# genome/pindel

Measured on AMD Instinct MI355X. Metric: one-end-anchored reads/sec through split-read search (close end + far end), higher is better.
Workload: dtype u64; 1 GPU; BASELINE configs[2]: synthetic 10000000 x 100 bp one-end-anchored reads on a chr20-shaped reference (62435964 bp), all SV types (D/SI/TD/INV/none), Pindel defaults -x 2 -a 1 -m 3 -u 0.02 -e 0.01 -E 0.95 -H 8; reads_per_gpu=10000000, reads_total=10000000, read_len=100, insert_size=500, parallelism=reads sharded over 1 GPU(s) (weak scaling), reference replicated, no collective

## Files before the change

pindel_amd/csrc/pg_kernels.hip:

```cpp
#include <hip/hip_runtime.h>
#include <stdint.h>
#include <stdlib.h>

#include "pg_device.h"
#include "pg_lane_masks.h"
#include "pg_eval_masks.h"
#include "pg_fold_step.h"

typedef unsigned long long u64;
typedef unsigned int u32;
typedef u32 u32x4 __attribute__((ext_vector_type(4)));
typedef u32 u32x8 __attribute__((ext_vector_type(8)));

struct PgKArgs { PgDevRef ref; PgDevParams prm; PgDevBatch B; uint32_t max_len, levels; };
template <typename T> struct KaGlobal { static __device__ __forceinline__ T of(unsigned long long v) { return (T)v; } };
template <typename E> struct KaGlobal<E *> {
    static __device__ __forceinline__ E *of(unsigned long long v) { return (E *)(__attribute__((address_space(1))) E *)v; }
};
template <typename T>
__device__ __forceinline__ T karg_load(int off)
{
    const auto k = __builtin_amdgcn_kernarg_segment_ptr();
    if (sizeof(T) == 8) {
        unsigned long long v;
// ... 125 lines not shown
template <int NB, int NS, typename Id, int mode, bool DEF, bool EXACT, int LEN>
constexpr bool pg_short_fold()
{
    if (!pg_short_masks<NB, NS, mode, DEF, EXACT, LEN>() || sizeof(Id) != 4) return false;
    if (LEN > 0) return true;
    if (NB == 2 && NS == 3 && mode == PG_MODE_FAR) return false;
    if (NB == 4 && (mode == PG_MODE_BOTH || mode == PG_MODE_CLOSE)) return false;
    if (NB == 8 && NS == 4 && (mode == PG_MODE_CLOSE || mode == PG_MODE_FAR)) return false;
    return true;
}
template <int NB, int NS, typename Id, int mode, bool DEF, bool EXACT, int LEN>
constexpr bool pg_open_pass()
{
    return LEN > 0 && NB <= 2 && PG_PASS(NB) == 64 && DEF && !EXACT;
}
#define PG_QUEUE_IDLE(nb) ((uint16_t)((64u * (nb)) << 1))
__device__ __forceinline__ int count_below(u64 m)
{
    return (int)__builtin_amdgcn_mbcnt_hi((u32)(m >> 32), __builtin_amdgcn_mbcnt_lo((u32)m, 0u));
}
__device__ __forceinline__ u64 bit_range(int lo, int hi)
{
    return low_bits(hi) & ~low_bits(lo);
}
__device__ __forceinline__ u64 funnel64(u32 w0, u32 w1, u32 w2, u32 s)
{
    u32 a = __builtin_amdgcn_alignbit(w1, w0, s);
    u32 b = __builtin_amdgcn_alignbit(w2, w1, s);
    return (u64)a | ((u64)b << 32);
}
// ... 13 lines not shown
    asm("s_lshl_b32 %0, %4, %5\n\ts_lshr_b32 %1, %4, %6\n\ts_add_u32 %0, %0, %2\n\ts_addc_u32 %1, %1, %3"
        : "=&s"(lo), "=&s"(hi) : "s"(blo), "s"(bhi), "s"(r), "n"(SHIFT), "n"(32 - SHIFT) : "scc");
    return KaGlobal<T *>::of((u64)lo | ((u64)hi << 32));
}

template <typename Id> struct IdFmt;
template <> struct IdFmt<u32> { static constexpr int RB = PG_REL_BITS_SMALL; };
template <> struct IdFmt<u64> { static constexpr int RB = PG_REL_BITS; };
template <typename Id>
__device__ __forceinline__ Id make_id(u32 rel, bool isB, u32 region)
{
    return (Id)rel | ((Id)(isB ? 1u : 0u) << IdFmt<Id>::RB) | ((Id)region << (IdFmt<Id>::RB + 1));
}

enum { QP_LO = 0, QP_HI = 1, QP_NN = 2, QP_OO = 3 };

template <int NB>
struct Query {
    const u64 *qp;
    bool allowF_, allowB_;
    bool cF_, cB_;
    bool first_ok_;
    bool o1_;
    __device__ __forceinline__ bool allowF() const { return allowF_; }
    __device__ __forceinline__ bool allowB() const { return allowB_; }
    __device__ __forceinline__ bool cF() const { return cF_; }
    __device__ __forceinline__ bool cB() const { return cB_; }
    __device__ __forceinline__ bool first_ok() const { return first_ok_; }
};
template <int NB> __device__ __forceinline__ u64 q_lo(const Query<NB> &Q, int b) { return Q.qp[QP_LO * NB + b]; }
// ... 19 lines not shown
template <> struct AccB<u64> {
    typedef uint4 T;
    static __device__ __forceinline__ void load(const void *base, int i, u32 &m1, u32 &m2, u32 &ok, u64 &id)
    {
        const uint4 st = ((const uint4 *)base)[i];
        m1 = st.x; m2 = st.y & 0xffffu; ok = st.y >> 16; id = (u64)st.z | ((u64)st.w << 32);
    }
    template <bool SF>
    static __device__ __forceinline__ void store(void *base, int i, u32 m1, u32 m2, u32 ok, u64 id)
    {
        static_assert(!SF, "the short form of the fold step has 32-bit ids");
        ((uint4 *)base)[i] = make_uint4(m1, m2 | (ok << 16), (u32)id, (u32)(id >> 32));
    }
};

template <int NB, typename Id>
struct Lds {
    uint4 bufA[68];
    uint2 bufB[PG_PASS(NB) * NB];
    uint2 hdrB[64];
    u64 ringB[3 * NB];
    typename AccB<Id>::T accB[NB > 1 ? 64 * (NB - 1) : 1];
    u64 qp[2 * 4 * NB];
    uint16_t queue[PG_PASS(NB)];
    uint8_t mm_tab[PG_MM_IN_WIN(NB) ? 4 : 64 * NB + 64];
    uint2 chr_tab[PG_CHR_TAB_N(NB)];
#ifdef PG_TIMING
    u64 t_last;
    u32 t_acc[12];
    u32 t_pad[2];
#endif
    uint4 win[PG_WIN_STATIC_WORDS(NB)];
};

struct Search {
    int len, T, M, add_mm, bps, min_perfect, thr;
    uint16_t *queue;
    uint4 *win;
// ... 25 lines not shown
#define PG_STOP_AT(S, k) do { asm volatile("s_nop 14\n\ts_nop %0\n\ts_nop %1" : : "n"((k) & 7), "n"((k) >> 3)); \
                              if (PG_STOP == (k) && uni(opaque(1))) { (S).stopped = 1u; return; } } while (0)
#define PG_STOPPED(S) do { if ((S).stopped) return; } while (0)
#define PG_STOP_AT_V(S, k, v) do { asm volatile("s_nop 14\n\ts_nop %0\n\ts_nop %1" : : "n"((k) & 7), "n"((k) >> 3)); \
                                 if (PG_STOP == (k) && uni(opaque(1))) { (S).stopped = 1u; return (v); } } while (0)
#define PG_STOPPED_V(S, v) do { if ((S).stopped) return (v); } while (0)
#else
#define PG_STOP_AT(S, k) ((void)0)
#define PG_STOPPED(S) ((void)0)
#define PG_STOP_AT_V(S, k, v) ((void)0)
#define PG_STOPPED_V(S, v) ((void)0)
#endif
#ifdef PG_DIAG
    u32 dg;
#endif
#if defined(PG_DIAG) && PG_DIAG == 3
#define PG_DG(S, sh) ((void)0)
#define PG_DC(S, sh) ((void)0)
#define PG_DC_IF(S, cond, sh) ((void)0)
#define PG_DN(S, sh, n) (const_cast<Search &>(S).dg += (u32)(n) << (sh))
#elif defined(PG_DIAG) && PG_DIAG == 2
#define PG_DG(S, sh) ((void)0)
#define PG_DC(S, sh) ((S).dg += 1u << (sh))
#define PG_DC_IF(S, cond, sh) ((S).dg += (cond) ? 1u << (sh) : 0u)
#define PG_DN(S, sh, n) ((void)0)
#elif defined(PG_DIAG)
#define PG_DG(S, sh) ((S).dg += 1u << (sh))
#define PG_DC(S, sh) ((void)0)
#define PG_DC_IF(S, cond, sh) ((void)0)
#define PG_DN(S, sh, n) ((void)0)
#else
#define PG_DG(S, sh) ((void)0)
#define PG_DC(S, sh) ((void)0)
#define PG_DC_IF(S, cond, sh) ((void)0)
#define PG_DN(S, sh, n) ((void)0)
#endif
    int cap_state;
    u32 sf;
    __device__ __forceinline__ bool want_cap() const { return (sf & 1u) != 0u; }
    __device__ __forceinline__ bool tierA() const { return (sf & 2u) != 0u; }
    __device__ __forceinline__ bool len_check() const { return (sf & 4u) != 0u; }
};

template <int NB, typename Id>
struct Acc {
    u32 m1, m2, ok;
    Id id;
    u32 a1, a2, aok;
    Id aid;
    u32 dirty;
    template <bool SF>
// ... 38 lines not shown
template <int NB>
__device__ __forceinline__ int chr_size_of(const PgDevRef &ref, const Search &S, int c)
{
    if (c < PG_CHR_TAB_N(NB)) {
        const int sz = uni((int)S.chr_tab[c].y);
        if (sz != 0) return sz;
    }
    return uni((int)KA(ref, chr_size)[c]);
}

template <int NB>
__device__ __forceinline__ void block_masks(const Query<NB> &Q, int b, bool comp,
                                            u64 rlo, u64 rhi, u64 rnn, u64 &mis, u64 &qn)
{
    const u64 qlo = q_lo<NB>(Q, b), qhi = q_hi<NB>(Q, b), qnn = q_nn<NB>(Q, b), qoo = q_oo<NB>(Q, b);
    u64 cm = comp ? ~0ull : 0ull;
    u64 x = rlo ^ qlo ^ cm;
    u64 y = rhi ^ qhi ^ cm;
    u64 d = x | y;
    mis = (d & ~qnn) | rnn | qoo;
    qn = qnn;
}

__device__ __forceinline__ void fetch_lds(const uint4 *win, int wbase, int q, bool rev,
                                          u64 &rlo, u64 &rhi, u64 &rnn)
{
    u32 rel = (u32)(q - wbase);
    u32 wi = rel >> 5, s = rel & 31u;
    uint4 w0 = win[wi], w1 = win[wi + 1], w2 = win[wi + 2];
    rlo = funnel64(w0.x, w1.x, w2.x, s);
    rhi = funnel64(w0.y, w1.y, w2.y, s);
    rnn = funnel64(w0.z, w1.z, w2.z, s);
    if (rev) { rlo = __brevll(rlo); rhi = __brevll(rhi); rnn = __brevll(rnn); }
}
__device__ __forceinline__ void fetch_lds_uniform(const uint4 *win, int wbase, int q, bool rev,
                                                  u64 &rlo, u64 &rhi, u64 &rnn)
// ... 75 lines not shown
            }
            u32 okc = pg_fs_verdict_b<SF>(bad, h.y);
            if (!SF && S.len_check()) okc = (u32)L >= ((h.y >> 24) & 0x7fu) ? okc : 0u;
            const Id cid = sizeof(Id) == 8 ? (Id)((u64)h.x | ((u64)(h.y & 0xffffffu) << 32)) : (Id)h.x;
            fold<Id>(m1, m2, wid, ok, k, cid, okc);
        }
        if (r == 0) { A.m1 = m1; A.m2 = m2; A.ok = ok; A.id = wid; }
        else {
            AccB<Id>::template store<SF>(S.accB, (r - 1) * 64 + lB, m1, m2, ok, wid);
            PG_DN(S, 27, 1);
            A.dirty |= 1u << r;
        }
    }
}

template <int NB, typename Id, bool MIXED, bool SM, bool SF, bool OP>
__device__ __forceinline__ void fold_candidates(const Search &S, const Query<NB> &Q, Acc<NB, Id> &A, int wbase,
                                                int origin, u32 region, int n, int lane, const Rings &R, int *ring_n)
{
    constexpr int EW = NB;
    PG_DG(const_cast<Search &>(S), 16);
    const u64 inm = low_bits(n);
    int p = 0;
    bool isB = MIXED ? false : Q.allowB();
    if (OP) {
        static_assert(!OP || PG_PASS(NB) == WAVE, "the open pass: one queue slot and one bufB slot per lane");
        const u32 e = S.queue[lane];
        if (MIXED) isB = e & 1u;
        p = wbase + (int)(e >> 1);
    } else if (lane_bit(inm)) {
        u32 e = S.queue[lane];
        if (MIXED) isB = e & 1u;
        p = wbase + (int)(e >> 1);
    }
    const bool comp = isB ? Q.cB() : Q.cF();
    int cum = 0, lvl0 = 0, kA = 0;
    int kk[NB];
    u32 m0lo = 0u, s0lo = 0u;
#pragma unroll
    for (int r = 0; r < NB; r++) kk[r] = 0;
    u64 needm = inm;
    const int alive = S.T > S.thr ? S.T : S.thr;
#pragma unroll
    for (int b = 0; b < NB; b++) {
        if (64 * b >= S.len) break;
        if (needm == 0ull) break;
        if (OP || lane_bit(needm)) {
            u64 rlo, rhi, rnn, m, s;
            int q = isB ? p - 64 * b - 63 : p + 64 * b;
            if (MIXED) fetch_lds(S.win, wbase, q, isB, rlo, rhi, rnn);
            else fetch_lds_uniform(S.win, wbase, q, isB, rlo, rhi, rnn);
            block_masks<NB>(Q, b, comp, rlo, rhi, rnn, m, s);
            const u64 lm = low_bits(S.len - 64 * b);
            m &= lm;
            s = (m ^ s) & lm;
            S.bufB[lane * EW + b] = make_uint2((u32)m, (u32)(m >> 32));
            cum += __popcll(m);
            if (b == 0) {
                lvl0 = __popcll(m & low_bits(S.bps));
                kA = __popc((u32)m & low32(S.bps + 16));
                m0lo = (u32)m;
                s0lo = (u32)s;
            }
#pragma unroll
            for (int r = 1; r < NB; r++)
                if (b <= r) kk[r] += __popcll(m & low_bits(S.bps + 64 * r - 64 * b));
        }
// ... 561 lines not shown
    PG_DG(const_cast<Search &>(S), 8);
    if (NS <= 4 && (S.ro & PG_RO_OK)) {
        constexpr int RNS = NS <= 3 ? 3 : 4;
        if (DUAL) seed_filter_ro<NB, 2, RNS>(S, Q.o1_, wide, lane, mF, mB);
        else if (kindB) seed_filter_ro<NB, 1, RNS>(S, Q.o1_, wide, lane, mF, mB);
        else seed_filter_ro<NB, 0, RNS>(S, Q.o1_, wide, lane, mF, mB);
        return;
    }
    const u32 jmask = S.jmask[wide ? 1 : 0];
    const u32 g0mask = jmask & low32(S.bps);
    int cap0 = (int)((S.depth >> (wide ? 24 : 16)) & 0xffu);
    if (cap0 > S.cap_state) cap0 = S.cap_state;
    seed_filter_run<NB, NS, DUAL>(S, Q, kindB, lane, jmask, g0mask, cap0, mF, mB);
}

template <int NB, int NS, typename Id, bool MIXED, bool W3, bool SM, bool SF, bool OP>
__device__ __forceinline__ void scan_impl(const PgDevRef &ref, Search &S,
                                          const Query<NB> &Q, Acc<NB, Id> &A, long long wo, int g0, int s, int e,
                                          int e_max, int xs, int xe, int origin, u32 region, int lane,
                                          u32 use_cache, u32 &cacheF, u32 &cacheB, u32 &cache_valid)
{
    if (!Q.first_ok() || s >= e) return;
    PG_STOP_AT(S, 33);
    const int k0 = (s - g0) >> PG_CHUNK_SHIFT, k1 = (e - 1 - g0) >> PG_CHUNK_SHIFT;
    for (int k = k0; k <= k1; k++) {
        const int cs = g0 + (k << PG_CHUNK_SHIFT);
        const int ns = s > cs ? s : cs;
        {
            const int ne = e < cs + (int)PG_CHUNK ? e : cs + (int)PG_CHUNK;
            if (ns >= xs && ne <= xe) continue;
        }
// ... 38 lines not shown
                    h++;
                    if (ballot64((mF | mB) != 0u) == 0ull) continue;
                    const u32 cnt = (u32)(__popc(mF) + __popc(mB));
                    const u32 incl = wave_scan(cnt);
                    slot = end + (int)(incl - cnt);
                    end += (int)read_lane(incl, 63);
                    pos0 = (u32)(64 * NB + 32 * word);
                    continue;
                }
                else if (end > 0) n = end;
                else break;
                S.nsurv += n;
                S.nsurv_total += (u32)n;
                PG_SYNC();
                PG_T(S, S.t_base);
                fold_candidates<NB, Id, MIXED, SM, SF, OP>(S, Q, A, wb, origin, region, n, lane, Rings{ false, 0, 0, 0, 0 }, nullptr);
                PG_STOPPED(S);
                PG_T(S, S.t_base + 1);
                slot -= n;
                end -= n;
                if (end == 0 && h == nh) break;
            }
            k += nh - 1;
            continue;
        }
        const int ne = e < cs + (int)PG_CHUNK ? e : cs + (int)PG_CHUNK;
        const int se = e_max < cs + (int)PG_CHUNK ? e_max : cs + (int)PG_CHUNK;
        PG_STOP_AT(S, 34);
        if (!(wo == S.win_wo && S.wbase == wb && se + 64 * NB <= S.win_hi))
            stage_window<NB>(ref, S, wo, wb, se + 64 * NB, lane);
        PG_STOP_AT(S, 13);
// ... 33 lines not shown
                S.queue[slot - base] = (uint16_t)((u32)(64 * NB + 32 * lane + bit) << 1);
                slot++;
            }
            while (mF == 0u && mB != 0u && slot < top) {
                const int bit = __ffs((int)mB) - 1;
                mB &= mB - 1u;
                S.queue[slot - base] = (uint16_t)(((u32)(64 * NB + 32 * lane + bit) << 1) | 1u);
                slot++;
            }
            const int n = total - base < PG_PASS(NB) ? total - base : PG_PASS(NB);
            S.nsurv += n;
            S.nsurv_total += (u32)n;
            PG_SYNC();
            PG_T(S, S.t_base);
            PG_STOP_AT(S, 16);
            fold_candidates<NB, Id, MIXED, SM, SF, OP>(S, Q, A, wb, origin, region, n, lane, Rings{ false, 0, 0, 0, 0 }, nullptr);
            PG_STOPPED(S);
            PG_T(S, S.t_base + 1);
        }
    }
}

template <int NB, int NS, typename Id, bool W3, bool SM, bool SF, bool OP>
__device__ __forceinline__ void scan_range(const PgDevRef &ref, Search &S,
                                           const Query<NB> &Q, Acc<NB, Id> &A, long long wo, int g0, int s, int e,
                                           int e_max, int xs, int xe, int origin, u32 region, int lane,
                                           u32 use_cache, u32 &cacheF, u32 &cacheB, u32 &cache_valid)
{
    g0 = uni(g0); s = uni(s); e = uni(e); e_max = uni(e_max); xs = uni(xs); xe = uni(xe); origin = uni(origin);
    if (Q.allowF() && Q.allowB())
        scan_impl<NB, NS, Id, true, W3, SM, SF, OP>(ref, S, Q, A, wo, g0, s, e, e_max, xs, xe, origin, region, lane,
                                    use_cache, cacheF, cacheB, cache_valid);
    else
        scan_impl<NB, NS, Id, false, false, SM, SF, OP>(ref, S, Q, A, wo, g0, s, e, e_max, xs, xe, origin, region, lane,
                                        use_cache, cacheF, cacheB, cache_valid);
}

template <int NB, int NS, typename Id, bool SM, bool SF, bool OP>
__device__ __forceinline__ void scan_staged(Search &S, const Query<NB> &Q, Acc<NB, Id> &A, int g0, int s, int e, int origin,
                                            int lane, u32 keep, u32 &cacheF, u32 &cacheB, u32 &cache_valid)
{
    const int wb = g0 - 64 * NB;
    PG_STOP_AT(S, 33);
    PG_STOP_AT(S, 34);
    PG_STOP_AT(S, 13);
    PG_STOP_AT(S, 37);
    u32 mF = 0u, mB = 0u, unused;
    if (Q.allowB()) seed_filter<NB, NS, false>(S, Q, true, false, lane, mB, unused);
    else seed_filter<NB, NS, false>(S, Q, false, false, lane, mF, unused);
    if (keep) { cacheF = mF; cacheB = mB; cache_valid = 1u; }
    PG_STOP_AT(S, 14);
    const u32 kb = Q.allowB() ? 1u : 0u;
    const int pbase = g0 + 32 * lane;
// ... 6 lines not shown
    for (int base = 0; base < total; base += PG_PASS(NB)) {
        PG_SYNC();
        const int top = base + PG_PASS(NB);
        while (m != 0u && slot < top) {
            const int bit = __ffs((int)m) - 1;
            m &= m - 1u;
            S.queue[slot - base] = (uint16_t)(((u32)(64 * NB + 32 * lane + bit) << 1) | kb);
            slot++;
        }
        const int n = total - base < PG_PASS(NB) ? total - base : PG_PASS(NB);
        S.nsurv += n;
        S.nsurv_total += (u32)n;
        PG_SYNC();
        PG_T(S, S.t_base);
        PG_STOP_AT(S, 16);
        fold_candidates<NB, Id, false, SM, SF, OP>(S, Q, A, wb, origin, 0u, n, lane, Rings{ false, 0, 0, 0, 0 }, nullptr);
        PG_STOPPED(S);
        PG_T(S, S.t_base + 1);
    }
}

struct RegionInfo {
    int chr;
    int origin;
    const pg_window *bd;
};

template <int NB, typename Id>
struct Eval {
    Id id[NB];
    u32 lo[NB];
    u64 startm[NB], brkm[NB];
    int n_runs, max_len;
    Id id_last;
};

template <int NB>
__device__ __forceinline__ u32 mm_of(const Search &S, int L)
{
    if (PG_MM_IN_WIN(NB)) return (S.win[L >> 2].w >> (8 * (L & 3))) & 0xffu;
    return S.mm_tab[L];
}

template <int NB, typename Id, bool SE, bool SF>
__device__ __forceinline__ void evaluate(Search &S, const Acc<NB, Id> &A, Eval<NB, Id> &E, int lane, int qmask = 15)
{
    static_assert(PG_MM_BREAKS < 64, "the short form's reach rule: no level of a point reaches 64");
    const u32 mm0 = mm_of<NB>(S, S.bps + lane);
    E.n_runs = 0;
    E.max_len = 0;
    E.id_last = 0;
    PG_DG(S, 24);
    u32 t1 = A.m1, t2 = A.m2, tok = A.ok;
    Id tid = A.id;
    if (S.tierA()) {
        u32 a1 = PG_BIG, a2 = PG_BIG, aok = pg_fs_none<SF>();
        Id aid = 0;
        if (lane < 16) { a1 = A.a1; a2 = A.a2; aok = A.aok; aid = A.aid; }
        if (qmask != 1) {
            PG_DC(S, 24);
            if (SF) S.bufA[lane] = make_uint4(A.a1, A.a2, (u32)A.aid, A.aok);
            else S.bufA[lane] = make_uint4(A.a1, A.a2 | (A.aok << 16), (u32)A.aid, (u32)((u64)A.aid >> 32));
            PG_SYNC();
            if (lane < 16) {
#pragma unroll
                for (int q = 1; q < 4; q++) {
                    if (!((qmask >> q) & 1)) continue;
                    const uint4 o = S.bufA[lane + 16 * q];
                    const Id oid = sizeof(Id) == 8 ? (Id)((u64)o.z | ((u64)o.w << 32)) : (Id)o.z;
                    if (SF) merge<Id>(a1, a2, aid, aok, o.x, o.y, oid, o.w);
// ... 115 lines not shown
            dst[0] = isB ? (u32)(p - L + 1) : (u32)(p + L - 1);
            dst[1] = (u32)L | ((u32)(S.bps + 64 * r + end_lane) << 16);
            dst[2] = E.lo[r] | ((isB ? PG_RUN_BACKWARD : 0u) << 8) | ((anti ? PG_RUN_ANTISENSE : 0u) << 8) |
                     ((u32)(chr & 0xffff) << 16);
        }
        written += __popcll(kept[r]);
    }
}

template <int NB>
__device__ __forceinline__ u64 request_planes(const PgDevBatch &B, uint32_t rid, int lane)
{
    const u32 pb = KA(B, plane_blocks);
    return (u32)lane < 8u * pb ? KA(B, planes)[(size_t)rid * 8u * pb + (u32)lane] : 0ull;
}
template <int NB>
__device__ __forceinline__ void store_planes(const PgDevBatch &B, u64 v, int lane, u64 *qp)
{
    const u32 pb = KA(B, plane_blocks);
    PG_SYNC();
    if ((u32)lane < 8u * pb) qp[pb == (u32)NB ? (u32)lane : ((u32)lane / pb) * NB + (u32)lane % pb] = v;
    PG_SYNC();
}

__device__ __forceinline__ u32 pool_alloc(const PgDevBatch &B, int n, int lane, u32 &fits)
{
    const u32 shard = blockIdx.x & (PG_POOL_SHARDS - 1u);
    u32 off = 0;
    if (n > 0 && lane == 0) off = atomicAdd(KA(B, pool_used) + shard * 16u, (u32)n);
    off = (u32)uni((int)off);
    fits = (u64)off + (u64)n <= (u64)KA(B, pool_shard_cap) ? 1u : 0u;
    return shard * KA(B, pool_shard_cap) + off;
}

template <int NB, int NS, typename Id, int mode, bool DEF, bool EXACT = false, int LEN = 0>
__device__ __forceinline__ void search_read(const PgDevRef &ref, const PgDevParams &prm, const PgDevBatch &B,
                                            Search &S, u64 *qplanes, const uint32_t rid, const int touch_next, const int lane,
                                            const u32 res_base, const u32 res_fits)
{
    constexpr bool OP = pg_open_pass<NB, NS, Id, mode, DEF, EXACT, LEN>();
#define PG_LANE (NB <= 2 && !OP ? lane_now() : opaque(lane))
    S.win_wo = -1;
    S.win_hi = S.wbase = 0;
    S.nsurv_total = 0u;
#ifdef PG_TIMING
    S.t_base = 1;
#endif
#ifdef PG_DIAG
    S.dg = 0u;
#endif
    S.cap_state = 255;
    S.sf = 0u;
#ifdef PG_STOP
    S.stopped = 0u;
#endif
// ... 32 lines not shown
        S.thr = (int)(F.lvl & 0xffffu);
        S.M = (int)((F.lvl >> 16) & 0xffu);
        S.T = (int)(F.lvl >> 24);
        S.depth = F.depth;
        S.jmask[0] = F.jmask0;
        S.ro = F.ro;
    }
    S.rid = rid;
    S.rp_lo = (u32)uni((int)(u32)(u64)(uintptr_t)rp);
    S.rp_hi = (u32)uni((int)(u32)((u64)(uintptr_t)rp >> 32));
    PG_STOP_AT(S, 10);
    if ((mode & PG_MODE_CLOSE) && (flags & PG_RF_CLOSE_OK)) {
        const int ss = (int)ra[2], se = (int)ra[3];
        if (ss < se) stage_window<NB>(ref, S, chr_wo, ss - 64 * NB, se + 64 * NB, lane, rp + uni(touch_next));
    }
    store_planes<NB>(B, planes_of_read, lane, qplanes);

    PG_T(S, 0);
#if defined(PG_STOP) && PG_STOP == 1
    if (uni(opaque(1))) return;
#endif
    int ja = 0, jb = 0, ex_stage = 0;
    auto ex_apply = [&](int to) __attribute__((always_inline)) {
        while (ex_stage < to) {
            ex_stage++;
            const int cut = ex_stage == 1 ? ja : jb;
            u64 *pl = qplanes + (ex_stage == 1 ? 0 : 4 * NB);
            if (cut > 0) {
                const int l = PG_LANE;
                u64 v = 0ull;
                if (l < 4 * NB) {
// ... 90 lines not shown
                    A.template reset<SF>();
                    S.cap_state = 255;
                    S.nsurv = 0;
                    nsurv_eval = 0;
                    ps = pe = 0;
                }
                if (att == 1 || att == 3) {
                    const u32 t0 = cr0, t1 = cr1;
                    const u32 tv = vr;
                    cr0 = co0; cr1 = co1; vr = vo;
                    co0 = t0; co1 = t1; vo = tv;
                }
                const bool own_grid = att == 0 && !shared_grid;
                PG_STOP_AT_V(S, 12, true);
                if (staged)
                    scan_staged<NB, NS, Id, SM, SF, OP>(S, Q, A, own_grid ? s1 : w1s, s1, e1, w1s, PG_LANE, shared_grid, cr0, cr1, vr);
                else
                scan_range<NB, NS, Id, !DEF, SM, SF, OP>(ref, S, Q, A, chr_wo, own_grid ? s1 : w1s, s1, e1, own_grid ? e1 : w1e, ps, pe, w1s, 0u,
                                   PG_LANE, (att == 1 || att == 2 ? 1u : 0u) | shared_grid, cr0, cr1, vr);
                PG_STOPPED_V(S, true);
                PG_STOP_AT_V(S, 19, true);
                ps = s1;
                pe = e1;
                if (S.nsurv != nsurv_eval) {
                    nsurv_eval = S.nsurv;
                    Eval<NB, Id> E;
                    PG_DC(S, 0);
                    evaluate<NB, Id, SE, SF>(S, A, E, PG_LANE);
                    PG_STOP_AT_V(S, 20, true);
                    close_max = uni(E.max_len);
                    if (uni(E.n_runs) > 0) {
                        u64 kept[NB];
                        n_close = uni(count_kept<NB, Id, SE>(E, true, kept));
                        if (n_close <= (int)PG_RES_CLOSE) {
                            close_base = res_base;
                            fits = res_fits;
                        } else
                            close_base = pool_alloc(B, n_close, lane, fits);
                        PG_DC(S, 20);
                        if (fits) emit_runs<NB, Id, SE>(S, true, false, chr, w1s, nullptr, E, kept, KA(B, pool) + close_base, PG_LANE);
                        const u64 idl = (u64)E.id_last;
                        const int pl = w1s + (int)(u32)(idl & ((1ull << IdFmt<Id>::RB) - 1ull));
                        close_last = ((idl >> IdFmt<Id>::RB) & 1ull) ? (u32)(pl - close_max + 1) : (u32)(pl + close_max - 1);
// ... 49 lines not shown
        Q.qp = qplanes + (flipped ? 4 * NB : 0);
        Q.o1_ = flipped != 0;
        Q.cF_ = flipped; Q.cB_ = !flipped;
        Q.allowF_ = Q.allowB_ = true;
        Q.first_ok_ = (flags & (flipped ? PG_RF_FIRST_OK_REV : PG_RF_FIRST_OK_FWD)) != 0u;
        if (Q.first_ok_) {
            u32x4 rc;
            asm volatile("s_load_dwordx4 %0, %1, 0x30\n\ts_waitcnt lgkmcnt(0)" : "=&s"(rc) : "s"(record_ptr<7>(KA(B, in), rid)));
            const int chr_size = (int)rc[0];
            S.jmask[1] = LEN > 0 ? pg_fixed_len_row((uint32_t)LEN).jmask1 : rc[3];
            PG_STOP_AT(S, 35);
            int far_bases = 0;
            auto far_update = [&](int origin, const pg_window *bdw, int qmask) {
                Eval<NB, Id> E;
                PG_DC(S, 4);
                evaluate<NB, Id, SE, SF>(S, A, E, PG_LANE, qmask);
                const int mx = uni(E.max_len);
                if (mx >= far_max) {
                    far_max = mx;
                    n_far = uni(E.n_runs);
                    far_base = 0;
                    if (n_far > 0) {
                        u64 kept[NB];
                        (void)count_kept<NB, Id, SE>(E, false, kept);
                        if (n_far <= (int)PG_RES_FAR) {
                            far_base = res_base + PG_RES_CLOSE;
                            fits &= res_fits;
                        } else {
                            u32 f2 = 1u;
                            far_base = pool_alloc(B, n_far, lane, f2);
                            fits &= f2;
// ... 6 lines not shown
            bool done = false;
            const pg_window *bd_all = KA(B, bd);
            if (bd_all && rc[1] != 0u) {
                const int nbd = (int)rc[1];
                const pg_window *bd = bd_all + rc[2];
                A.template reset<SF>();
                S.cap_state = 255;
                S.nsurv = 0;
                for (int w = 0; w < nbd; w++) {
                    const pg_window bw = bd[w];
                    const int st = bw.start < 0 ? bw.end - 1 : bw.start;
                    const bool own_chr = uni(bw.chr_id) == chr;
                    const int csz = own_chr ? chr_size : chr_size_of<NB>(ref, S, uni(bw.chr_id));
                    const int s = st < 0 ? 0 : st, e = bw.end > csz ? csz : bw.end;
                    far_bases += (e > s ? e - s : 0) + 2 * len;
                    scan_range<NB, NS, Id, !DEF, SM, SF, OP>(ref, S, Q, A, own_chr ? chr_wo : chr_word_off_of<NB>(ref, S, uni(bw.chr_id)), s, s, e, e, 0, 0, st,
                                       (u32)w, PG_LANE, false, unused0, unused1, unused_valid);
                    PG_STOPPED(S);
                }
                if (S.nsurv > 0) far_update(0, bd, 15);
                done = far_max + close_max >= len;
            }
            if (!done) {
                const int center = (int)close_last;
                const int k_mri = PRM(max_range_index, PG_DEF_MAX_RANGE_INDEX);
                const u32 k_spacer = PRM(spacer, PG_DEF_SPACER);
                const int maxspan = 64 << (2 * k_mri);
                const int origin = center - maxspan;
                const int g0 = center - (int)PG_CHUNK / 2;
                const u32 reach = (u32)maxspan + k_spacer;
                const bool noclip = reach >= k_spacer && (u32)center > reach && (u32)chr_size > reach && (u32)center < (u32)chr_size - reach;
// ... 59 lines not shown
                                    S.queue[slot] = (uint16_t)((u32)(64 * NB + 32 * lane + bit) << 1);
                                    slot++;
                                }
                                while (mB != 0u) {
                                    const int bit = __ffs((int)mB) - 1;
                                    mB &= mB - 1u;
                                    S.queue[slot] = (uint16_t)(((u32)(64 * NB + 32 * lane + bit) << 1) | 1u);
                                    slot++;
                                }
                                S.nsurv += total;
                                S.nsurv_total += (u32)total;
                                PG_SYNC();
                                PG_STOP_AT(S, 27);
                                int ring_n[3];
                                PG_T(S, 7);
                                fold_candidates<NB, Id, true, SM, SF, OP>(S, Q, A, wb, origin, 0u, total, lane,
                                                              Rings{ true, rs[0], re[0], rs[1], re[1] }, ring_n);
                                PG_STOPPED(S);
                                PG_STOP_AT(S, 30);
                                PG_T(S, 8);
                                for (int r = 0; r <= R; r++) {
                                    if (uni(ring_n[r]) > 0) {
                                        u64 longm[NB];
#pragma unroll
                                        for (int k = 0; k < NB; k++) longm[k] = read_lane(S.ringB[r * NB + k], 0);
                                        fold_tier_b<NB, Id, SM, SF>(S, Q, A, longm, lane);
                                        far_update(origin, nullptr, r == 0 ? 1 : (r == 1 ? 3 : 15));
                                    }
                                    if (far_max + close_max >= len) {
                                        done = true;
                                        ps = rs[r];
                                        pe = re[r];
                                        break;
                                    }
                                }
                                nsurv_eval = S.nsurv;
                            }
                        }
                    }
                    PG_STOP_AT(S, 31);
                }
                int span = 64 << (2 * r_first);
                for (int r = r_first; r <= k_mri && !done; r++, span *= 4) {
                    int s, e;
                    range_of(span, s, e);
                    if (s < e) {
                        scan_range<NB, NS, Id, !DEF, SM, SF, OP>(ref, S, Q, A, chr_wo, g0, s, e, emax, ps, pe, origin, 0u, PG_LANE, true,
                                           cacheF, cacheB, cache_valid);
                        PG_STOPPED(S);
                        if (ps < pe) {
                            ps = s < ps ? s : ps;
                            pe = e > pe ? e : pe;
                        } else {
                            ps = s; pe = e;
                        }
                    }
                    if (S.nsurv != nsurv_eval) {
                        nsurv_eval = S.nsurv;
                        far_update(origin, nullptr, 15);
                    }
                    if (far_max + close_max >= len) break;
                }
// ... 736 lines not shown
```

pindel_amd/csrc/pg_search_kernel_body.h:

```cpp
    __shared__ Lds<NB, Id> lds;
    const int lane = threadIdx.x;
    if (PG_WIN_DYN_BYTES(NB) != 0u) {
        extern __shared__ uint4 pg_dyn_lds[];
        if ((const char *)pg_dyn_lds != (const char *)&lds + sizeof(lds)) __builtin_trap();
    }
    if (PG_MM_IN_WIN(NB)) {
        for (int w = lane; w < 16 * NB + 16; w += WAVE) {
            u32 v = 0u;
#pragma unroll
            for (int k = 0; k < 4; k++) v |= (u32)max_mismatch_at(prm.mm_bp, 4 * w + k) << (8 * k);
            lds.win[w].w = v;
        }
    } else
        for (int L = lane; L < 64 * NB + 64; L += WAVE) lds.mm_tab[L] = (uint8_t)max_mismatch_at(prm.mm_bp, L);
    if (lane < PG_CHR_TAB_N(NB) && lane < ref.n_chr) {
        const u64 wo = ref.chr_word_off[lane];
        lds.chr_tab[lane] = make_uint2((u32)wo, (wo >> 32) == 0ull ? ref.chr_size[lane] : 0u);
    }
    PG_SYNC();
    Search S;
    S.queue = lds.queue;
    S.win = lds.win;
    S.bufA = lds.bufA;
    S.bufB = lds.bufB;
    S.hdrB = lds.hdrB;
    S.ringB = lds.ringB;
    S.accB = lds.accB;
    S.mm_tab = lds.mm_tab;
    S.chr_tab = lds.chr_tab;
    u64 *qplanes = lds.qp;
    if (lane < 8 * NB) qplanes[lane] = 0ull;
    if (pg_open_pass<NB, NS, Id, mode, DEF, false, LEN>() && lane < PG_PASS(NB)) lds.queue[lane] = PG_QUEUE_IDLE(NB);
#ifdef PG_TIMING
    S.t_acc = lds.t_acc;
    S.t_last = &lds.t_last;
    if (lane == 0) {
        for (int k = 0; k < 12; k++) S.t_acc[k] = 0u;
        *S.t_last = __builtin_readcyclecounter();
    }
    S.t_base = 1;
#endif

    uint32_t part = blockIdx.x % PG_N_XCD, tried = 0;
    while (tried < PG_N_XCD) {
        const uint32_t n = KA(B, n_reads);
        const uint32_t claim = KA(B, claim);
// ... 44 lines not shown
```

Before: 581.9 million reads/s.

## Precompute bit-reversed query planes and tree-merge quarter accumulators in evaluate

After: 588.2 million reads/s (median of 6 runs). 1.01x the previous value.

```diff
diff --git a/pindel_amd/csrc/pg_kernels.hip b/pindel_amd/csrc/pg_kernels.hip
--- a/pindel_amd/csrc/pg_kernels.hip
+++ b/pindel_amd/csrc/pg_kernels.hip
@@ -6,6 +6,7 @@
 #include "pg_lane_masks.h"
 #include "pg_eval_masks.h"
 #include "pg_fold_step.h"
+#include "pg_pass_forms.h"
 
 typedef unsigned long long u64;
 typedef unsigned int u32;
@@ -163,6 +164,16 @@
 {
     return LEN > 0 && NB <= 2 && PG_PASS(NB) == 64 && DEF && !EXACT;
 }
+template <int NB, int NS, typename Id, int mode, bool DEF, bool EXACT, int LEN>
+constexpr bool pg_rev_mismatch()
+{
+    return LEN > 0 && NB == 2 && DEF && !EXACT;
+}
+template <int NB, int NS, typename Id, int mode, bool DEF, bool EXACT, int LEN>
+constexpr bool pg_tree_merge()
+{
+    return LEN > 0 && NB <= 2 && PG_PASS(NB) == 64 && pg_short_fold<NB, NS, Id, mode, DEF, EXACT, LEN>();
+}
 #define PG_QUEUE_IDLE(nb) ((uint16_t)((64u * (nb)) << 1))
 __device__ __forceinline__ int count_below(u64 m)
 {
@@ -206,6 +217,7 @@
 }
 
 enum { QP_LO = 0, QP_HI = 1, QP_NN = 2, QP_OO = 3 };
+#define PG_QP_REV(nb) (2 * 4 * (nb))
 
 template <int NB>
 struct Query {
@@ -255,14 +267,14 @@
     }
 };
 
-template <int NB, typename Id>
+template <int NB, typename Id, int QPX = 2>
 struct Lds {
     uint4 bufA[68];
     uint2 bufB[PG_PASS(NB) * NB];
     uint2 hdrB[64];
     u64 ringB[3 * NB];
     typename AccB<Id>::T accB[NB > 1 ? 64 * (NB - 1) : 1];
-    u64 qp[2 * 4 * NB];
+    u64 qp[QPX * 4 * NB];
     uint16_t queue[PG_PASS(NB)];
     uint8_t mm_tab[PG_MM_IN_WIN(NB) ? 4 : 64 * NB + 64];
     uint2 chr_tab[PG_CHR_TAB_N(NB)];
@@ -318,7 +330,13 @@
 #ifdef PG_DIAG
     u32 dg;
 #endif
-#if defined(PG_DIAG) && PG_DIAG == 3
+#if defined(PG_DIAG) && PG_DIAG == 4
+#define PG_DG(S, sh) ((void)0)
+#define PG_DC(S, sh) ((void)0)
+#define PG_DC_IF(S, cond, sh) ((void)0)
+#define PG_DN(S, sh, n) ((void)0)
+#define PG_DK(S, sh) (const_cast<Search &>(S).dg += 1u << (sh))
+#elif defined(PG_DIAG) && PG_DIAG == 3
 #define PG_DG(S, sh) ((void)0)
 #define PG_DC(S, sh) ((void)0)
 #define PG_DC_IF(S, cond, sh) ((void)0)
@@ -339,6 +357,9 @@
 #define PG_DC_IF(S, cond, sh) ((void)0)
 #define PG_DN(S, sh, n) ((void)0)
 #endif
+#ifndef PG_DK
+#define PG_DK(S, sh) ((void)0)
+#endif
     int cap_state;
     u32 sf;
     __device__ __forceinline__ bool want_cap() const { return (sf & 1u) != 0u; }
@@ -407,12 +428,24 @@
                                             u64 rlo, u64 rhi, u64 rnn, u64 &mis, u64 &qn)
 {
     const u64 qlo = q_lo<NB>(Q, b), qhi = q_hi<NB>(Q, b), qnn = q_nn<NB>(Q, b), qoo = q_oo<NB>(Q, b);
-    u64 cm = comp ? ~0ull : 0ull;
-    u64 x = rlo ^ qlo ^ cm;
-    u64 y = rhi ^ qhi ^ cm;
-    u64 d = x | y;
-    mis = (d & ~qnn) | rnn | qoo;
+    mis = pg_pf_mismatch(rlo, rhi, rnn, qlo, qhi, qnn, qoo, comp);
     qn = qnn;
+}
+template <int NB>
+__device__ __forceinline__ void block_masks_at(const Query<NB> &Q, const u64 *qb, int b, bool comp,
+                                               u64 rlo, u64 rhi, u64 rnn, u64 &mis, u64 &qn)
+{
+    mis = pg_pf_mismatch(rlo, rhi, rnn, qb[QP_LO * NB + b], qb[QP_HI * NB + b], qb[QP_NN * NB + b], qb[QP_OO * NB + b], comp);
+    qn = q_nn<NB>(Q, b);
+}
+__device__ __forceinline__ void fetch_lds_plain(const uint4 *win, int wbase, int q, u64 &rlo, u64 &rhi, u64 &rnn)
+{
+    u32 rel = (u32)(q - wbase);
+    u32 wi = rel >> 5, s = rel & 31u;
+    uint4 w0 = win[wi], w1 = win[wi + 1], w2 = win[wi + 2];
+    rlo = funnel64(w0.x, w1.x, w2.x, s);
+    rhi = funnel64(w0.y, w1.y, w2.y, s);
+    rnn = funnel64(w0.z, w1.z, w2.z, s);
 }
 
 __device__ __forceinline__ void fetch_lds(const uint4 *win, int wbase, int q, bool rev,
@@ -518,7 +551,7 @@
     }
 }
 
-template <int NB, typename Id, bool MIXED, bool SM, bool SF, bool OP>
+template <int NB, typename Id, bool MIXED, bool SM, bool SF, bool OP, bool RM>
 __device__ __forceinline__ void fold_candidates(const Search &S, const Query<NB> &Q, Acc<NB, Id> &A, int wbase,
                                                 int origin, u32 region, int n, int lane, const Rings &R, int *ring_n)
 {
@@ -538,6 +571,7 @@
         p = wbase + (int)(e >> 1);
     }
     const bool comp = isB ? Q.cB() : Q.cF();
+    const u64 *const qrm = Q.qp + (RM && isB ? PG_QP_REV(NB) : 0);
     int cum = 0, lvl0 = 0, kA = 0;
     int kk[NB];
     u32 m0lo = 0u, s0lo = 0u;
@@ -549,12 +583,23 @@
     for (int b = 0; b < NB; b++) {
         if (64 * b >= S.len) break;
         if (needm == 0ull) break;
+        PG_DK(S, MIXED ? 12 : (isB ? 0 : 6));
         if (OP || lane_bit(needm)) {
             u64 rlo, rhi, rnn, m, s;
             int q = isB ? p - 64 * b - 63 : p + 64 * b;
+            if (RM) {
+                fetch_lds_plain(S.win, wbase, q, rlo, rhi, rnn);
+                block_masks_at<NB>(Q, qrm, b, comp, rlo, rhi, rnn, m, s);
+                if (MIXED) m = isB ? __brevll(m) : m;
+                else if (uni((int)isB)) {
+                    asm volatile("" : "+v"(m));
+                    m = __brevll(m);
+                }
+            } else {
             if (MIXED) fetch_lds(S.win, wbase, q, isB, rlo, rhi, rnn);
             else fetch_lds_uniform(S.win, wbase, q, isB, rlo, rhi, rnn);
             block_masks<NB>(Q, b, comp, rlo, rhi, rnn, m, s);
+            }
             const u64 lm = low_bits(S.len - 64 * b);
             m &= lm;
             s = (m ^ s) & lm;
@@ -1146,7 +1191,7 @@
     seed_filter_run<NB, NS, DUAL>(S, Q, kindB, lane, jmask, g0mask, cap0, mF, mB);
 }
 
-template <int NB, int NS, typename Id, bool MIXED, bool W3, bool SM, bool SF, bool OP>
+template <int NB, int NS, typename Id, bool MIXED, bool W3, bool SM, bool SF, bool OP, bool RM>
 __device__ __forceinline__ void scan_impl(const PgDevRef &ref, Search &S,
                                           const Query<NB> &Q, Acc<NB, Id> &A, long long wo, int g0, int s, int e,
                                           int e_max, int xs, int xe, int origin, u32 region, int lane,
@@ -1215,7 +1260,7 @@
                 S.nsurv_total += (u32)n;
                 PG_SYNC();
                 PG_T(S, S.t_base);
-                fold_candidates<NB, Id, MIXED, SM, SF, OP>(S, Q, A, wb, origin, region, n, lane, Rings{ false, 0, 0, 0, 0 }, nullptr);
+                fold_candidates<NB, Id, MIXED, SM, SF, OP, RM>(S, Q, A, wb, origin, region, n, lane, Rings{ false, 0, 0, 0, 0 }, nullptr);
                 PG_STOPPED(S);
                 PG_T(S, S.t_base + 1);
                 slot -= n;
@@ -1279,14 +1324,14 @@
             PG_SYNC();
             PG_T(S, S.t_base);
             PG_STOP_AT(S, 16);
-            fold_candidates<NB, Id, MIXED, SM, SF, OP>(S, Q, A, wb, origin, region, n, lane, Rings{ false, 0, 0, 0, 0 }, nullptr);
+            fold_candidates<NB, Id, MIXED, SM, SF, OP, RM>(S, Q, A, wb, origin, region, n, lane, Rings{ false, 0, 0, 0, 0 }, nullptr);
             PG_STOPPED(S);
             PG_T(S, S.t_base + 1);
         }
     }
 }
 
-template <int NB, int NS, typename Id, bool W3, bool SM, bool SF, bool OP>
+template <int NB, int NS, typename Id, bool W3, bool SM, bool SF, bool OP, bool RM>
 __device__ __forceinline__ void scan_range(const PgDevRef &ref, Search &S,
                                            const Query<NB> &Q, Acc<NB, Id> &A, long long wo, int g0, int s, int e,
                                            int e_max, int xs, int xe, int origin, u32 region, int lane,
@@ -1294,14 +1339,14 @@
 {
     g0 = uni(g0); s = uni(s); e = uni(e); e_max = uni(e_max); xs = uni(xs); xe = uni(xe); origin = uni(origin);
     if (Q.allowF() && Q.allowB())
-        scan_impl<NB, NS, Id, true, W3, SM, SF, OP>(ref, S, Q, A, wo, g0, s, e, e_max, xs, xe, origin, region, lane,
+        scan_impl<NB, NS, Id, true, W3, SM, SF, OP, RM>(ref, S, Q, A, wo, g0, s, e, e_max, xs, xe, origin, region, lane,
                                     use_cache, cacheF, cacheB, cache_valid);
     else
-        scan_impl<NB, NS, Id, false, false, SM, SF, OP>(ref, S, Q, A, wo, g0, s, e, e_max, xs, xe, origin, region, lane,
+        scan_impl<NB, NS, Id, false, false, SM, SF, OP, RM>(ref, S, Q, A, wo, g0, s, e, e_max, xs, xe, origin, region, lane,
                                         use_cache, cacheF, cacheB, cache_valid);
 }
 
-template <int NB, int NS, typename Id, bool SM, bool SF, bool OP>
+template <int NB, int NS, typename Id, bool SM, bool SF, bool OP, bool RM>
 __device__ __forceinline__ void scan_staged(Search &S, const Query<NB> &Q, Acc<NB, Id> &A, int g0, int s, int e, int origin,
                                             int lane, u32 keep, u32 &cacheF, u32 &cacheB, u32 &cache_valid)
 {
@@ -1338,7 +1383,7 @@
         PG_SYNC();
         PG_T(S, S.t_base);
         PG_STOP_AT(S, 16);
-        fold_candidates<NB, Id, false, SM, SF, OP>(S, Q, A, wb, origin, 0u, n, lane, Rings{ false, 0, 0, 0, 0 }, nullptr);
+        fold_candidates<NB, Id, false, SM, SF, OP, RM>(S, Q, A, wb, origin, 0u, n, lane, Rings{ false, 0, 0, 0, 0 }, nullptr);
         PG_STOPPED(S);
         PG_T(S, S.t_base + 1);
     }
@@ -1366,7 +1411,7 @@
     return S.mm_tab[L];
 }
 
-template <int NB, typename Id, bool SE, bool SF>
+template <int NB, typename Id, bool SE, bool SF, bool TM = false>
 __device__ __forceinline__ void evaluate(Search &S, const Acc<NB, Id> &A, Eval<NB, Id> &E, int lane, int qmask = 15)
 {
     static_assert(PG_MM_BREAKS < 64, "the short form's reach rule: no level of a point reaches 64");
@@ -1377,7 +1422,26 @@
     PG_DG(S, 24);
     u32 t1 = A.m1, t2 = A.m2, tok = A.ok;
     Id tid = A.id;
-    if (S.tierA()) {
+    if (S.tierA() && qmask != 1) PG_DK(S, qmask == 3 ? 18 : 23);
+    if (TM && S.tierA()) {
+        static_assert(!TM || (SF && sizeof(Id) == 4), "the tree merge moves the short fold step's four words");
+        u32 a1 = A.a1, a2 = A.a2, aok = A.aok;
+        u32 aid = (u32)A.aid;
+        if (qmask != 1) {
+            PG_DC(S, 24);
+            const int at = opaque(lane) << 2;
+            auto take = [&](int up) {
+                const u32 b1 = (u32)__builtin_amdgcn_ds_bpermute(at + 4 * up, (int)a1), b2 = (u32)__builtin_amdgcn_ds_bpermute(at + 4 * up, (int)a2),
+                          bid = (u32)__builtin_amdgcn_ds_bpermute(at + 4 * up, (int)aid), bok = (u32)__builtin_amdgcn_ds_bpermute(at + 4 * up, (int)aok);
+                merge<u32>(a1, a2, aid, aok, b1, b2, bid, bok);
+            };
+            take(16);
+            if (qmask == 15) take(32);
+        }
+        const bool q0 = lane < 16;
+        a1 = q0 ? a1 : PG_BIG; a2 = q0 ? a2 : PG_BIG; aok = q0 ? aok : pg_fs_none<SF>(); aid = q0 ? aid : 0u;
+        merge<Id>(t1, t2, tid, tok, a1, a2, (Id)aid, aok);
+    } else if (S.tierA()) {
         u32 a1 = PG_BIG, a2 = PG_BIG, aok = pg_fs_none<SF>();
         Id aid = 0;
         if (lane < 16) { a1 = A.a1; a2 = A.a2; aok = A.aok; aid = A.aid; }
@@ -1523,12 +1587,16 @@
     const u32 pb = KA(B, plane_blocks);
     return (u32)lane < 8u * pb ? KA(B, planes)[(size_t)rid * 8u * pb + (u32)lane] : 0ull;
 }
-template <int NB>
+template <int NB, bool RM = false>
 __device__ __forceinline__ void store_planes(const PgDevBatch &B, u64 v, int lane, u64 *qp)
 {
     const u32 pb = KA(B, plane_blocks);
     PG_SYNC();
-    if ((u32)lane < 8u * pb) qp[pb == (u32)NB ? (u32)lane : ((u32)lane / pb) * NB + (u32)lane % pb] = v;
+    if ((u32)lane < 8u * pb) {
+        const u32 at = pb == (u32)NB ? (u32)lane : ((u32)lane / pb) * NB + (u32)lane % pb;
+        qp[at] = v;
+        if (RM) qp[PG_QP_REV(NB) + at] = __brevll(v);
+    }
     PG_SYNC();
 }
 
@@ -1548,6 +1616,8 @@
                                             const u32 res_base, const u32 res_fits)
 {
     constexpr bool OP = pg_open_pass<NB, NS, Id, mode, DEF, EXACT, LEN>();
+    constexpr bool RM = pg_rev_mismatch<NB, NS, Id, mode, DEF, EXACT, LEN>();
+    constexpr bool TM = pg_tree_merge<NB, NS, Id, mode, DEF, EXACT, LEN>();
 #define PG_LANE (NB <= 2 && !OP ? lane_now() : opaque(lane))
     S.win_wo = -1;
     S.win_hi = S.wbase = 0;
@@ -1610,7 +1680,7 @@
         const int ss = (int)ra[2], se = (int)ra[3];
         if (ss < se) stage_window<NB>(ref, S, chr_wo, ss - 64 * NB, se + 64 * NB, lane, rp + uni(touch_next));
     }
-    store_planes<NB>(B, planes_of_read, lane, qplanes);
+    store_planes<NB, RM>(B, planes_of_read, lane, qplanes);
 
     PG_T(S, 0);
 #if defined(PG_STOP) && PG_STOP == 1
@@ -1731,9 +1801,9 @@
                 const bool own_grid = att == 0 && !shared_grid;
                 PG_STOP_AT_V(S, 12, true);
                 if (staged)
-                    scan_staged<NB, NS, Id, SM, SF, OP>(S, Q, A, own_grid ? s1 : w1s, s1, e1, w1s, PG_LANE, shared_grid, cr0, cr1, vr);
+                    scan_staged<NB, NS, Id, SM, SF, OP, RM>(S, Q, A, own_grid ? s1 : w1s, s1, e1, w1s, PG_LANE, shared_grid, cr0, cr1, vr);
                 else
-                scan_range<NB, NS, Id, !DEF, SM, SF, OP>(ref, S, Q, A, chr_wo, own_grid ? s1 : w1s, s1, e1, own_grid ? e1 : w1e, ps, pe, w1s, 0u,
+                scan_range<NB, NS, Id, !DEF, SM, SF, OP, RM>(ref, S, Q, A, chr_wo, own_grid ? s1 : w1s, s1, e1, own_grid ? e1 : w1e, ps, pe, w1s, 0u,
                                    PG_LANE, (att == 1 || att == 2 ? 1u : 0u) | shared_grid, cr0, cr1, vr);
                 PG_STOPPED_V(S, true);
                 PG_STOP_AT_V(S, 19, true);
@@ -1743,7 +1813,7 @@
                     nsurv_eval = S.nsurv;
                     Eval<NB, Id> E;
                     PG_DC(S, 0);
-                    evaluate<NB, Id, SE, SF>(S, A, E, PG_LANE);
+                    evaluate<NB, Id, SE, SF, TM>(S, A, E, PG_LANE);
                     PG_STOP_AT_V(S, 20, true);
                     close_max = uni(E.max_len);
                     if (uni(E.n_runs) > 0) {
@@ -1823,7 +1893,7 @@
             auto far_update = [&](int origin, const pg_window *bdw, int qmask) {
                 Eval<NB, Id> E;
                 PG_DC(S, 4);
-                evaluate<NB, Id, SE, SF>(S, A, E, PG_LANE, qmask);
+                evaluate<NB, Id, SE, SF, TM>(S, A, E, PG_LANE, qmask);
                 const int mx = uni(E.max_len);
                 if (mx >= far_max) {
                     far_max = mx;
@@ -1860,7 +1930,7 @@
                     const int csz = own_chr ? chr_size : chr_size_of<NB>(ref, S, uni(bw.chr_id));
                     const int s = st < 0 ? 0 : st, e = bw.end > csz ? csz : bw.end;
                     far_bases += (e > s ? e - s : 0) + 2 * len;
-                    scan_range<NB, NS, Id, !DEF, SM, SF, OP>(ref, S, Q, A, own_chr ? chr_wo : chr_word_off_of<NB>(ref, S, uni(bw.chr_id)), s, s, e, e, 0, 0, st,
+                    scan_range<NB, NS, Id, !DEF, SM, SF, OP, RM>(ref, S, Q, A, own_chr ? chr_wo : chr_word_off_of<NB>(ref, S, uni(bw.chr_id)), s, s, e, e, 0, 0, st,
                                        (u32)w, PG_LANE, false, unused0, unused1, unused_valid);
                     PG_STOPPED(S);
                 }
@@ -1950,7 +2020,7 @@
                                 PG_STOP_AT(S, 27);
                                 int ring_n[3];
                                 PG_T(S, 7);
-                                fold_candidates<NB, Id, true, SM, SF, OP>(S, Q, A, wb, origin, 0u, total, lane,
+                                fold_candidates<NB, Id, true, SM, SF, OP, RM>(S, Q, A, wb, origin, 0u, total, lane,
                                                               Rings{ true, rs[0], re[0], rs[1], re[1] }, ring_n);
                                 PG_STOPPED(S);
                                 PG_STOP_AT(S, 30);
@@ -1981,7 +2051,7 @@
                     int s, e;
                     range_of(span, s, e);
                     if (s < e) {
-                        scan_range<NB, NS, Id, !DEF, SM, SF, OP>(ref, S, Q, A, chr_wo, g0, s, e, emax, ps, pe, origin, 0u, PG_LANE, true,
+                        scan_range<NB, NS, Id, !DEF, SM, SF, OP, RM>(ref, S, Q, A, chr_wo, g0, s, e, emax, ps, pe, origin, 0u, PG_LANE, true,
                                            cacheF, cacheB, cache_valid);
                         PG_STOPPED(S);
                         if (ps < pe) {
diff --git a/pindel_amd/csrc/pg_pass_forms.h b/pindel_amd/csrc/pg_pass_forms.h
--- /dev/null
+++ b/pindel_amd/csrc/pg_pass_forms.h
@@ -0,0 +1,93 @@
+#ifndef PG_PASS_FORMS_H
+#define PG_PASS_FORMS_H
+#include <stdint.h>
+#include "pg_fold_step.h"
+
+#define PG_PF_FN PG_FS_FN
+
+PG_PF_FN uint64_t pg_pf_brev64(uint64_t v)
+{
+#if defined(__HIP_DEVICE_COMPILE__)
+    return __brevll(v);
+#else
+    uint64_t r = 0ull;
+    for (int i = 0; i < 64; i++) r |= ((v >> i) & 1ull) << (63 - i);
+    return r;
+#endif
+}
+PG_PF_FN uint64_t pg_pf_low_bits(int n)
+{
+    return n >= 64 ? ~0ull : (n <= 0 ? 0ull : ((1ull << n) - 1ull));
+}
+
+PG_PF_FN uint64_t pg_pf_mismatch(uint64_t rlo, uint64_t rhi, uint64_t rnn, uint64_t qlo, uint64_t qhi, uint64_t qnn, uint64_t qoo, bool comp)
+{
+    const uint64_t cm = comp ? ~0ull : 0ull;
+    const uint64_t x = rlo ^ qlo ^ cm;
+    const uint64_t y = rhi ^ qhi ^ cm;
+    const uint64_t d = x | y;
+    return (d & ~qnn) | rnn | qoo;
+}
+PG_PF_FN void pg_pf_finish(uint64_t &m, uint64_t &s, uint64_t qnn, int bases)
+{
+    const uint64_t lm = pg_pf_low_bits(bases);
+    m &= lm;
+    s = (m ^ qnn) & lm;
+}
+
+struct PgPfPlanes {
+    uint64_t lo, hi, nn, oo;
+};
+PG_PF_FN PgPfPlanes pg_pf_reversed(const PgPfPlanes &q)
+{
+    PgPfPlanes r;
+    r.lo = pg_pf_brev64(q.lo); r.hi = pg_pf_brev64(q.hi); r.nn = pg_pf_brev64(q.nn); r.oo = pg_pf_brev64(q.oo);
+    return r;
+}
+PG_PF_FN void pg_pf_block_ref_reversed(uint64_t rlo, uint64_t rhi, uint64_t rnn, const PgPfPlanes &q, bool comp, bool isB, int bases,
+                                       uint64_t &m, uint64_t &s)
+{
+    if (isB) { rlo = pg_pf_brev64(rlo); rhi = pg_pf_brev64(rhi); rnn = pg_pf_brev64(rnn); }
+    m = pg_pf_mismatch(rlo, rhi, rnn, q.lo, q.hi, q.nn, q.oo, comp);
+    pg_pf_finish(m, s, q.nn, bases);
+}
+PG_PF_FN void pg_pf_block_mis_reversed(uint64_t rlo, uint64_t rhi, uint64_t rnn, const PgPfPlanes &q, const PgPfPlanes &qr, bool comp,
+                                       bool isB, int bases, uint64_t &m, uint64_t &s)
+{
+    const PgPfPlanes &u = isB ? qr : q;
+    m = pg_pf_mismatch(rlo, rhi, rnn, u.lo, u.hi, u.nn, u.oo, comp);
+    if (isB) m = pg_pf_brev64(m);
+    pg_pf_finish(m, s, q.nn, bases);
+}
+
+template <typename Id>
+struct PgPfQuarter {
+    uint32_t m1, m2;
+    Id id;
+    uint32_t v;
+};
+template <typename Id>
+PG_PF_FN void pg_pf_merge(PgPfQuarter<Id> &a, const PgPfQuarter<Id> &b)
+{
+    pg_fs_merge<Id>(a.m1, a.m2, a.id, a.v, b.m1, b.m2, b.id, b.v);
+}
+template <typename Id>
+PG_PF_FN PgPfQuarter<Id> pg_pf_quarters_chain(const PgPfQuarter<Id> *q, int qmask)
+{
+    PgPfQuarter<Id> a = q[0];
+    for (int k = 1; k < 4; k++)
+        if ((qmask >> k) & 1) pg_pf_merge<Id>(a, q[k]);
+    return a;
+}
+template <typename Id>
+PG_PF_FN PgPfQuarter<Id> pg_pf_quarters_tree(const PgPfQuarter<Id> *q, int qmask)
+{
+    PgPfQuarter<Id> a = q[0], c = q[2];
+    if (qmask == 1) return a;
+    pg_pf_merge<Id>(a, q[1]);
+    pg_pf_merge<Id>(c, q[3]);
+    if (qmask == 15) pg_pf_merge<Id>(a, c);
+    return a;
+}
+
+#endif
diff --git a/pindel_amd/csrc/pg_search_kernel_body.h b/pindel_amd/csrc/pg_search_kernel_body.h
--- a/pindel_amd/csrc/pg_search_kernel_body.h
+++ b/pindel_amd/csrc/pg_search_kernel_body.h
@@ -1,4 +1,5 @@
-    __shared__ Lds<NB, Id> lds;
+    constexpr int QPX = pg_rev_mismatch<NB, NS, Id, mode, DEF, false, LEN>() ? 4 : 2;
+    __shared__ Lds<NB, Id, QPX> lds;
     const int lane = threadIdx.x;
     if (PG_WIN_DYN_BYTES(NB) != 0u) {
         extern __shared__ uint4 pg_dyn_lds[];
@@ -29,7 +30,7 @@
     S.mm_tab = lds.mm_tab;
     S.chr_tab = lds.chr_tab;
     u64 *qplanes = lds.qp;
-    if (lane < 8 * NB) qplanes[lane] = 0ull;
+    if (lane < 4 * QPX * NB) qplanes[lane] = 0ull;
     if (pg_open_pass<NB, NS, Id, mode, DEF, false, LEN>() && lane < PG_PASS(NB)) lds.queue[lane] = PG_QUEUE_IDLE(NB);
 #ifdef PG_TIMING
     S.t_acc = lds.t_acc;
```
